# Robinatp/YOLO_Tensorflow

Measured on AMD Instinct MI355X. Metric: images_per_sec, higher is better.
Workload: dtype bf16; 1 GPU; YOLOv3 416x416 batch=32 per GPU, bf16: conv stack + head decode + threshold + TF-NMS; global_batch=32, input=uint8 NHWC resident in HBM, weights=seeded synthetic darknet stream (seed 0), parallelism=dp1

## Files before the change

yolo_tensorflow_amd/csrc/kernels.h:

```cpp
#pragma once
#ifndef OUT_STORE_AUX
#define OUT_STORE_AUX 16
#endif
#ifndef HALO_LOAD_AUX
#define HALO_LOAD_AUX 0
#endif
#ifndef RES_LOAD_AUX
#define RES_LOAD_AUX 0
#endif
#include <hip/hip_runtime.h>
#include <stdint.h>
typedef unsigned out_u32x4 __attribute__((ext_vector_type(4)));
__device__ __forceinline__ void out_store16_at(const void *base, unsigned byte_off, unsigned x, unsigned y, unsigned z, unsigned w)
{
#if defined(__HIP_DEVICE_COMPILE__)
    __amdgpu_buffer_rsrc_t r = __builtin_amdgcn_make_buffer_rsrc((void *)base, 0, 0x80000000u, 0x00020000);
    __builtin_amdgcn_raw_buffer_store_b128(out_u32x4{x, y, z, w}, r, byte_off, 0, OUT_STORE_AUX);
#endif
}

typedef uint16_t bf16_t;
struct fp8_t { uint8_t b; };
struct f16_t { uint16_t b; };
enum { DT_BF16 = 0, DT_F32 = 1, DT_FP8 = 2, DT_F16 = 3 };
// ... 88 lines not shown
};
bool conv_stem_pair_ok(const StemPairArgs &a);
hipError_t launch_conv_stem_pair(const StemPairArgs &a, hipStream_t s);
bool conv_c8_direct_pair_ok(const ConvArgs &a);
hipError_t launch_conv_c8_direct_pair(const ConvArgs &a, hipStream_t s);
hipError_t launch_conv_fp8(const ConvArgs &a, int cfg, hipStream_t s);
hipError_t launch_conv_diag(const ConvArgs &a, hipStream_t s);
struct StemArgs {
    const void *in; int in_stride;
    const uint8_t *in_u8; float in_scale, in_mul, in_add;
    const void *w0; const float *b0; int Kpad0, C0, act0;
    const void *w1; const float *b1; int Kpad1, C1, act1;
    void *out; int out_stride;
    int dt;
    const void *w2; const float *b2; int Kpad2, C2, act2;
    void *out2; int out2_stride;
    int N, H, W, Ho, Wo;
    const void *zeros;
};
bool conv_stem_ok(const StemArgs &a);
hipError_t launch_conv_stem(const StemArgs &a, hipStream_t s);
struct HaloArgs {
    const void *in; int in_stride;
    const void *w; const float *b; int Kpad, Cin, Cout, act;
    const void *res; int res_stride;
    void *out; int out_stride;
    int N, H, W;
    int dt;
};
bool conv_halo_ok(const HaloArgs &a);
hipError_t launch_conv_halo(const HaloArgs &a, hipStream_t s);
bool conv_s2_ok(const HaloArgs &a);
hipError_t launch_conv_s2(const HaloArgs &a, hipStream_t s);
struct BlockArgs {
    const void *x; int x_stride;
    const void *w1; const float *b1; int Kpad1, act1;
    const void *w2; const float *b2; int Kpad2, act2;
    void *out; int out_stride;
    int N, H, W, C, Cmid;
    int dt;
};
bool conv_resblock_ok(const BlockArgs &a);
hipError_t launch_conv_resblock(const BlockArgs &a, hipStream_t s);
hipError_t launch_conv_f32(const ConvArgs &a, hipStream_t s);

hipError_t launch_preprocess(const void *img, int fmt , int n, int hw, float scale,
                             void *out, int out_dt, int out_stride, hipStream_t s, float post_mul = 1.0f, float post_add = 0.0f);
hipError_t launch_resize_u8(const uint8_t *img, int h, int w, int s_out, void *out, int out_dt,
                            int out_stride, int out_c, hipStream_t s, float post_scale = 1.0f, float post_add = 0.0f);
hipError_t launch_resize_cv2_u8(const uint8_t *img, int h, int w, int oh, int ow, int swap_rb, float divisor, float *out, hipStream_t s);
struct ImgDesc { unsigned long long offset; int h, w; };
enum { FIT_STRETCH = 0, FIT_LETTERBOX = 1, FIT_CV2 = 2, FIT_CV2_BGR = 3 };
hipError_t launch_fit_images(const uint8_t *pixels, size_t bytes, const ImgDesc *d_descs, int n, int fit, int S, void *out, int out_dt,
                             int out_stride, float post_mul, float post_add, hipStream_t s);
__host__ __device__ inline void letterbox_dims(int netw, int neth, int w, int h, int *new_w, int *new_h)
{
    if (((float)netw / w) < ((float)neth / h)) { *new_w = netw; *new_h = (h * netw) / w; } else { *new_h = neth; *new_w = (w * neth) / h; }
}
__host__ __device__ inline float fit_unit_value(int fit, unsigned v)
{
    if (fit == FIT_STRETCH) return (float)v / 255.0f;
    if (fit == FIT_LETTERBOX) return (float)((double)v / 255.);
    return (float)v;
}
hipError_t launch_upsample2x(const TView &in, const TView &out, int bilinear, hipStream_t s);
hipError_t launch_maxpool(const TView &in, const TView &out, int size, int stride, int pad, hipStream_t s);
// ... 82 lines not shown
```

yolo_tensorflow_amd/csrc/yolo_api.cpp:

```cpp
#include "yolo_ctx.h"

extern "C" {

yolo_ctx *yolo_create(const yolo_config *cfg, char *err, size_t err_len)
{
    auto bail = [&](yolo_ctx *c, const std::string &m) -> yolo_ctx * { if (err && err_len) snprintf(err, err_len, "%s", m.c_str()); if (c) yolo_destroy(c); return nullptr; };
    if (!cfg || cfg->struct_size != sizeof(yolo_config)) return bail(nullptr, "yolo_create: bad yolo_config (struct_size)");
    if (cfg->max_batch < 1) return bail(nullptr, "yolo_create: max_batch < 1");
    if (cfg->dtype != YOLO_BF16 && cfg->dtype != YOLO_FP32 && cfg->dtype != YOLO_FP8 && cfg->dtype != YOLO_FP16 && cfg->dtype != YOLO_FP16X2) return bail(nullptr, "yolo_create: dtype");
    yolo_ctx *c = new yolo_ctx();
    c->device = cfg->device; c->max_batch = cfg->max_batch; c->dtype = cfg->dtype; c->semantics = cfg->semantics;
    c->decode = cfg->decode; c->keep_layers = cfg->keep_layers;
    int ndev = 0;
    if (hipGetDeviceCount(&ndev) != hipSuccess || ndev < 1) return bail(c, "yolo_create: no HIP device (this library has no CPU fallback)");
    if (hipSetDevice(c->device) != hipSuccess) return bail(c, "yolo_create: hipSetDevice failed");
    if (cfg->stream) c->stream = (hipStream_t)cfg->stream;
    else { if (hipStreamCreate(&c->stream) != hipSuccess) return bail(c, "yolo_create: hipStreamCreate failed"); c->own_stream = true; }
    std::vector<Section> secs; std::string perr;
    c->cfg_text = cfg->cfg_text ? cfg->cfg_text : "";
    if (!parse_cfg(cfg->cfg_text, secs, perr)) return bail(c, perr);
    if (build_plan(c, secs) != YOLO_OK) return bail(c, c->err);
    if (allocate(c) != YOLO_OK) return bail(c, c->err);
    resolve_scales(c);
    return c;
// ... 17 lines not shown

const char *yolo_last_error(const yolo_ctx *c) { return c ? c->err.c_str() : g_op_err.c_str(); }

size_t yolo_weights_count(const yolo_ctx *c) { return c ? c->weights_count : 0; }

int yolo_input_size(const yolo_ctx *c, int *h, int *w, int *ch) { if (!c) return YOLO_ERR_INVALID; if (h) *h = c->in_h; if (w) *w = c->in_w; if (ch) *ch = c->in_c; return YOLO_OK; }
int yolo_num_rows(const yolo_ctx *c) { return c ? c->rows : YOLO_ERR_INVALID; }
int yolo_num_attrs(const yolo_ctx *c) { return c ? c->attrs : YOLO_ERR_INVALID; }
int yolo_num_classes(const yolo_ctx *c) { return !c ? YOLO_ERR_INVALID : c->cls_layer >= 0 ? c->layers[c->cls_layer].C : c->attrs - 5; }
int yolo_num_layers(const yolo_ctx *c) { return c ? (int)c->layers.size() : YOLO_ERR_INVALID; }
int yolo_head_geometry(const yolo_ctx *c, int head, int *kind, int *grid, int *anchors, int *row_offset)
{
    if (!c || head < 0) return YOLO_ERR_INVALID;
    int k = 0;
    for (auto &L : c->layers) {
        if (L.type != L_YOLO && L.type != L_REGION && L.type != L_DETECT) continue;
        if (k++ != head) continue;
        if (kind) *kind = L.type == L_REGION ? 1 : L.type == L_DETECT ? 2 : 0;
        if (grid) *grid = L.H;
        if (anchors) *anchors = L.na;
        if (row_offset) *row_offset = L.row_off;
        return YOLO_OK;
    }
    return YOLO_ERR_INVALID;
}
double yolo_conv_flops(const yolo_ctx *c) { return c ? c->conv_flops : 0; }
double yolo_conv_bytes(const yolo_ctx *c, int n)
{
    if (!c) return 0;
    double b = 0;
    for (auto &L : c->layers) if (L.type == L_CONV) {
        TView in = view_of(c, L.in[0]);
        const double ie = (double)dt_size(L.in_dt), oe = (double)dt_size(L.out.dt);
        if (!L.stem && !L.stem_tail && !L.blk) b += (double)n * in.h * in.w * L.cin * ie;
        if (!L.stem_skip && !L.blk_skip && !L.pstem_skip) b += (double)n * L.H * L.W * L.filters * oe;
        b += (double)L.filters * L.cin * L.size * L.size * ie;
    }
    return b;
}

int yolo_darknet_boxes(yolo_ctx *c, int w, int h, float thresh, int relative, float *records, int cap, int *count)
{
    return yolo_darknet_boxes_at(c, 0, w, h, thresh, relative, records, cap, count);
}

int yolo_darknet_boxes_at(yolo_ctx *c, int image, int w, int h, float thresh, int relative, float *records, int cap, int *count)
{
    if (!c || !count) return YOLO_ERR_INVALID;
    if (int r = need_detector(c, "yolo_darknet_boxes")) return r;
    if (c->last_n < 1 || !c->det_valid) return fail(c, YOLO_ERR_STATE, "yolo_darknet_boxes needs a yolo_forward* pass first");
    if (image < 0 || image >= c->last_n) return fail(c, YOLO_ERR_INVALID, "image %d outside the last forward's batch of %d", image, c->last_n);
    if (w < 1 || h < 1 || cap < 0 || (cap > 0 && !records)) return fail(c, YOLO_ERR_INVALID, "bad image size / capacity");
    HIPCK(c, hipSetDevice(c->device));
    if (!c->d_dn_rec) {
        HIPCK(c, hipMalloc((void **)&c->d_dn_rec, (size_t)c->rows * c->attrs * 4));
        HIPCK(c, hipMalloc((void **)&c->d_dn_src, (size_t)c->rows * 4));
        HIPCK(c, hipMalloc((void **)&c->d_dn_count, 4));
    }
    DnBoxesArgs a; memset(&a, 0, sizeof a);
    a.det = c->d_det + (size_t)image * c->rows * c->attrs; a.attrs = c->attrs;
    for (size_t li = 0; li < c->layers.size(); ++li) {
        const Layer &L = c->layers[li];
        if (L.type != L_YOLO && L.type != L_REGION && L.type != L_DETECT) continue;
        if (a.nheads == 8) return fail(c, YOLO_ERR_UNSUPPORTED, "more than 8 heads");
        if (L.type == L_DETECT) {
            if (a.nheads) return fail(c, YOLO_ERR_UNSUPPORTED, "a [detection] head next to other heads");
            a.raw = (const float *)c->layers[li - 1].out.ptr + (size_t)image * c->layers[li - 1].out.stride; a.side = L.side; a.classes = L.classes; a.sqr = L.sqr;
            a.kind[0] = 2; a.grid[0] = L.side; a.na[0] = L.na; a.off[0] = L.row_off; a.nheads = 1;
// ... 58 lines not shown
    HIPCK(c, hipMemcpyAsync(out, c->d_dn_last, need * 4, hipMemcpyDeviceToHost, c->stream)); HIPCK(c, hipStreamSynchronize(c->stream));
    return YOLO_OK;
}

int yolo_last_layer_output(yolo_ctx *c, float *out, size_t out_floats) { return yolo_last_layer_output_batch(c, 1, out, out_floats); }

int yolo_head_raw(yolo_ctx *c, int head, int n, float *out, size_t out_floats)
{
    if (!c || !out || head < 0) return YOLO_ERR_INVALID;
    if (int r = need_detector(c, "yolo_head_raw")) return r;
    if (c->last_n < 1 || n < 1 || n > c->last_n) return fail(c, YOLO_ERR_STATE, "yolo_head_raw of %d images but the last forward ran %d", n, c->last_n);
    int k = 0;
    for (size_t li = 1; li < c->layers.size(); ++li) {
        const Layer &L = c->layers[li];
        if (L.type != L_YOLO && L.type != L_REGION && L.type != L_DETECT) continue;
        if (k++ != head) continue;
        const Layer &P = c->layers[li - 1];
        const size_t px = (size_t)n * P.H * P.W, need = px * P.C;
        if (out_floats < need) return fail(c, YOLO_ERR_INVALID, "output buffer too small (%zu < %zu floats)", out_floats, need);
        if (P.out.dt != DT_F32 || !P.out.ptr) return fail(c, YOLO_ERR_STATE, "internal: head conv output is not fp32");
        HIPCK(c, hipSetDevice(c->device));
        HIPCK(c, hipMemcpy2DAsync(out, (size_t)P.C * 4, P.out.ptr, (size_t)P.out.stride * 4, (size_t)P.C * 4, px, hipMemcpyDeviceToHost, c->stream));
        HIPCK(c, hipStreamSynchronize(c->stream));
        return YOLO_OK;
    }
    return fail(c, YOLO_ERR_INVALID, "no detection head %d", head);
}

int yolo_synchronize(yolo_ctx *c) { if (!c) return YOLO_ERR_INVALID; HIPCK(c, hipStreamSynchronize(c->stream)); return YOLO_OK; }

int yolo_layer_output(yolo_ctx *c, int index, int n, float *out, size_t out_floats, int *dims_out)
{
    if (!c) return YOLO_ERR_INVALID;
    if (!c->keep_layers) return fail(c, YOLO_ERR_STATE, "yolo_layer_output needs keep_layers=1");
    if (index < 0 || index >= (int)c->layers.size() || n < 1 || n > c->last_n) return fail(c, YOLO_ERR_INVALID, "bad layer index / n");
    const Layer &L = c->layers[index];
    if (dims_out) { dims_out[0] = L.H; dims_out[1] = L.W; dims_out[2] = L.C; }
    size_t need = (size_t)n * L.H * L.W * L.C;
    if (!out) return YOLO_OK;
    if (out_floats < need) return fail(c, YOLO_ERR_INVALID, "output buffer too small");
    HIPCK(c, hipSetDevice(c->device));
    float *tmp = nullptr; HIPCK(c, hipMalloc((void **)&tmp, need * 4));
    TView v = L.out; v.n = n;
    float vs = 1.f;
    if (v.dt == DT_FP8) {
        vs = c->eff_scale[index];
        if (vs != vs) { hipFree(tmp); return fail(c, YOLO_ERR_UNSUPPORTED, "layer %d concatenates tensors with different fp8 scales; read its sources", index); }
    }
    hipError_t e = hipSuccess;
    float *wide = nullptr;
    if (L.pair && v.dt == DT_F16) {
        const int cp = roundup(L.C, 32);
        e = hipMalloc((void **)&wide, (size_t)n * L.H * L.W * cp * 4);
        if (e == hipSuccess) e = launch_split_to_f32(v.ptr, v.stride, cp, wide, cp, (size_t)n * L.H * L.W, c->stream);
        v.ptr = wide; v.stride = cp; v.dt = DT_F32;
    }
    if (e == hipSuccess) e = launch_to_f32(v, tmp, c->stream, vs);
    if (e == hipSuccess) e = hipMemcpyAsync(out, tmp, need * 4, hipMemcpyDeviceToHost, c->stream);
    if (e == hipSuccess) e = hipStreamSynchronize(c->stream);
    hipFree(tmp); if (wide) hipFree(wide);
    if (e != hipSuccess) return fail(c, YOLO_ERR_HIP, "layer_output: %s", hipGetErrorString(e));
    return YOLO_OK;
}

}
```

yolo_tensorflow_amd/csrc/yolo_ctx.h:

```cpp
#pragma once
#include "../../include/yolo_hip.h"
#include "kernels.h"

#include <algorithm>
#include <cmath>
#include <cstdarg>
#include <cstdio>
#include <cstdlib>
#include <cstring>
#include <map>
#include <string>
#include <vector>

namespace yolo_impl {

enum LType { L_CONV, L_SHORTCUT, L_ROUTE, L_UPSAMPLE, L_MAXPOOL, L_REORG, L_YOLO, L_REGION, L_DETECT, L_LOCAL, L_AVGPOOL, L_SOFTMAX };

struct Section { std::string type; std::map<std::string, std::string> kv; };

struct Layer {
    LType type;
    int H = 0, W = 0, C = 0;
    std::vector<int> in;
    int filters = 0, size = 0, stride = 1, pad = 0, bn = 0, act = ACT_LINEAR;
    int cin = 0, cin_pad = 0, kpad = 0, cout_pad = 0;
    void *d_w = nullptr; float *d_b = nullptr; float *d_sc = nullptr;
    void *d_wf = nullptr;
    int in_dt = DT_BF16;
    int store_dt = DT_BF16;
    bool pair = false;
    int tile_cfg = -1;
    int residual_from = -2;
    bool head = false;
    float *d_obj = nullptr;
    bool stem_skip = false, stem = false;
    bool pstem_skip = false, pstem = false;
    bool blk_skip = false, blk = false;
    bool stem_tail = false;
    bool halo = false;
    bool s2 = false;
    bool fc = false; int fc_h = 0, fc_w = 0, fc_c = 0;
    bool s2d7 = false;
    int side = 0, sqr = 0;
    int tail_layer = -1, fused_into = -1; bool tail_on = false;
    bool noop = false;
    std::vector<int> copy_inputs;
    std::vector<int> copy_offsets;
    int psize = 0, pstride = 0, ppad = 0;
    int na = 0, classes = 0, row_off = 0;
    std::vector<float> anchors;
    int groups = 1; float temperature = 1.f; bool pool_fused = false; bool cost = false;
    int storage = -1; int ch_off = 0;
    TView out;
};

struct Storage { int def = 1 << 30, last = -1; size_t bytes = 0; int phys = -1; int stride = 0; int dt = DT_BF16; bool persistent = false; };


}
using namespace yolo_impl;

struct yolo_ctx {
    std::string err, cfg_text;
    int device = 0;
    hipStream_t stream = nullptr; bool own_stream = false;
    int max_batch = 1, dtype = YOLO_BF16, semantics = YOLO_SEM_TF, decode = YOLO_DECODE_RATIO, keep_layers = 0;
    int in_h = 0, in_w = 0, in_c = 0;
    std::vector<Layer> layers;
    std::vector<Storage> storages;
    std::vector<void *> phys; std::vector<size_t> phys_bytes;
    TView input;
    void *d_zeros = nullptr;
    void *d_stage = nullptr; size_t stage_bytes = 0;
// ... 82 lines not shown
```

yolo_tensorflow_amd/csrc/yolo_plan.cpp:

```cpp
#include "yolo_ctx.h"

namespace yolo_impl {

bool parse_cfg(const char *text, std::vector<Section> &out, std::string &err)
{
    std::string s(text ? text : "");
    size_t pos = 0;
    while (pos <= s.size()) {
        size_t e = s.find('\n', pos); if (e == std::string::npos) e = s.size();
        std::string line = s.substr(pos, e - pos); pos = e + 1;
        size_t a = line.find_first_not_of(" \t\r"); if (a == std::string::npos) continue;
        size_t b = line.find_last_not_of(" \t\r"); line = line.substr(a, b - a + 1);
        if (line[0] == '#' || line[0] == ';') continue;
        if (line[0] == '[') {
            size_t r = line.find(']'); if (r == std::string::npos) { err = "cfg: unterminated section " + line; return false; }
            Section sec; sec.type = line.substr(1, r - 1); out.push_back(sec);
        } else {
            size_t eq = line.find('='); if (eq == std::string::npos || out.empty()) { err = "cfg: bad line '" + line + "'"; return false; }
            std::string k = line.substr(0, eq), v = line.substr(eq + 1);
            auto trim = [](std::string &t) { size_t x = t.find_first_not_of(" \t"); size_t y = t.find_last_not_of(" \t"); t = x == std::string::npos ? "" : t.substr(x, y - x + 1); };
            trim(k); trim(v); out.back().kv[k] = v;
        }
    }
    if (out.empty() || (out[0].type != "net" && out[0].type != "network")) { err = "cfg: first section must be [net]"; return false; }
// ... 221 lines not shown
        }
    if (ctx16 && !c->keep_layers && NL >= 2 && (double)c->max_batch * c->in_h * c->in_w * 8 * 2 < 2147483648.0) {
        const Layer &A = c->layers[0], &B = c->layers[1];
        if (A.type == L_CONV && B.type == L_CONV && uses[0] == 1 && B.in[0] == 0 && A.size == 3 && A.stride == 1 && A.pad == 1 && A.cin == 3 &&
            A.filters == 32 && B.size == 3 && B.stride == 2 && B.pad == 1 && B.filters == 64 && !A.head && !B.head && B.residual_from < -1 &&
            is16(A.in_dt) && A.store_dt == A.in_dt && B.in_dt == A.in_dt && B.store_dt == A.in_dt && !c->in_pair && !A.pair && !B.pair) {
            c->layers[0].stem_skip = true; c->layers[1].stem = true;
            if (NL >= 3) {
                const Layer &T = c->layers[2];
                if (T.type == L_CONV && !T.fc && T.in[0] == 1 && T.size == 1 && T.stride == 1 && T.pad == 0 && T.filters == 32 && !T.head && T.residual_from < -1 &&
                    T.in_dt == A.in_dt && T.store_dt == A.in_dt && !T.pair)
                    c->layers[2].stem_tail = true;
            }
        }
    }
    if (c->split() && !c->keep_layers && NL >= 2 && c->in_pair && !getenv("YOLO_NO_PAIR_STEM")) {
        const Layer &A = c->layers[0], &B = c->layers[1];
        if (A.type == L_CONV && B.type == L_CONV && uses[0] == 1 && B.in[0] == 0 && A.size == 3 && A.stride == 1 && A.pad == 1 && A.cin == 3 && A.bn == B.bn &&
            (A.filters == 32) && B.size == 3 && B.stride == 2 && B.pad == 1 && B.filters == 64 && !A.head && !B.head && A.residual_from < -1 && B.residual_from < -1 &&
            A.pair && B.pair && c->in_h % 2 == 0 && c->in_w % 2 == 0 && A.kpad >= 216 && B.kpad == 576) {
            c->layers[0].pstem_skip = true; c->layers[1].pstem = true;
        }
    }
    if (ctx16 && !getenv("YOLO_NO_HALO"))
        for (int i = 1; i < NL; ++i) {
            Layer &L = c->layers[i];
            if (L.type == L_CONV && !L.head && !L.stem && !L.stem_skip && !L.stem_tail && !L.blk && L.size == 3 && L.stride == 1 && L.pad == 1 && L.cin == 32 && L.filters == 64 &&
                is16(L.in_dt) && L.store_dt == L.in_dt && (L.residual_from < 0 || c->layers[L.residual_from].store_dt == L.in_dt) && !L.pair && !c->pair_of(L.in[0]))
                L.halo = true;
            if (L.type == L_CONV && !L.head && !L.stem && !L.stem_skip && !L.stem_tail && !L.blk && !L.blk_skip && L.size == 3 && L.stride == 2 && L.pad == 1 && L.cin == 64 &&
                L.filters == 128 && L.residual_from < -1 && is16(L.in_dt) && L.store_dt == L.in_dt && !L.pair && !c->pair_of(L.in[0]) && !getenv("YOLO_NO_S2"))
                L.s2 = true;
        }
    if (ctx16 && !c->keep_layers) {
        for (int i = 0; i + 1 < NL; ++i) {
            Layer &P = c->layers[i];
            if (P.type != L_CONV || P.fc || P.head || P.stem || P.stem_skip || P.stem_tail || P.blk || P.s2 || P.halo || (P.filters != 128 && P.filters != 256)) continue;
            if (c->split() && (P.pair || c->pair_of(P.in[0]))) continue;
            int o = i;
            if (P.residual_from >= -1) o = i + 1;
            const int j = o + 1;
            if (j >= NL) continue;
            Layer &T = c->layers[j];
            if (T.type == L_CONV && !T.fc && T.in[0] == o && T.size == 1 && T.stride == 1 && T.pad == 0 && T.filters * 2 == P.filters && !T.head &&
                T.residual_from < -1 && !T.stem_tail && !T.blk_skip && T.in_dt == P.in_dt && !T.pair) { P.tail_layer = j; T.fused_into = i; }
            else if (T.type == L_CONV && !T.fc && T.head && T.in[0] == o && uses[o] == 1 && T.size == 1 && T.stride == 1 && T.pad == 0 && P.filters == 256 && T.filters <= 256 &&
                     P.size == 3 && P.residual_from < -1 && T.act == ACT_LINEAR && T.in_dt == P.in_dt && (T.in_dt == DT_BF16 || T.in_dt == DT_F16) && j + 1 < NL && c->layers[j + 1].type == L_YOLO) { P.tail_layer = j; T.fused_into = i; }
        }
    }
    std::vector<int> place_route(NL, -1), place_off(NL, 0);
    for (int i = 0; i < NL; ++i) {
        Layer &L = c->layers[i];
        if (L.type != L_ROUTE || L.in.size() < 2) continue;
        int off = 0;
        for (int j : L.in) {
            int cj = j < 0 ? c->in_c : c->layers[j].C;
            const int gran = L.pair ? 32 : gran_of(L.store_dt);
            bool ok = j >= 0 && place_route[j] < 0 && c->layers[j].type != L_ROUTE && !c->layers[j].head &&
                      c->layers[j].type != L_YOLO && c->layers[j].type != L_REGION && c->layers[j].type != L_DETECT && (cj % gran == 0) && (off % gran == 0) &&
                      c->layers[j].type != L_SOFTMAX && !c->layers[j].cost && !(c->layers[j].type == L_AVGPOOL && c->layers[j].store_dt != L.store_dt);
            if (ok && c->layers[j].type == L_CONV && j + 1 < NL && c->layers[j + 1].noop && c->layers[j + 1].type == L_SHORTCUT) ok = false;
            if (ok) { place_route[j] = i; place_off[j] = L.pair ? 2 * off : off; }
            else { L.copy_inputs.push_back(j); L.copy_offsets.push_back(off); }
            off += cj;
        }
    }
// ... 2 lines not shown
        c->storages.push_back(s); return (int)c->storages.size() - 1;
    };
    for (int i = 0; i < NL; ++i) {
        Layer &L = c->layers[i];
        if (L.type == L_ROUTE && L.in.size() >= 2) {
            L.storage = new_storage(L.pair ? pair_width(L.C) : roundup(L.C, gran_of(L.store_dt)), L.store_dt, (size_t)c->max_batch * L.H * L.W, c->keep_layers); L.ch_off = 0;
        }
    }
    for (int i = 0; i < NL; ++i) {
        Layer &L = c->layers[i];
        if (L.type == L_YOLO || L.type == L_REGION || L.type == L_DETECT) { L.noop = true; L.storage = c->layers[i - 1].storage; L.ch_off = c->layers[i - 1].ch_off; continue; }
        if (L.type == L_ROUTE && L.in.size() == 1) { L.noop = true; int j = L.in[0]; if (j < 0) return fail(c, YOLO_ERR_UNSUPPORTED, "route to network input"); L.storage = c->layers[j].storage; L.ch_off = c->layers[j].ch_off; continue; }
        if (L.type == L_ROUTE) continue;
        if (L.stem_skip || L.pstem_skip) { L.noop = true; continue; }
        if (L.type == L_SOFTMAX) { L.storage = new_storage(L.C, DT_F32, (size_t)c->max_batch, true); continue; }
        if (place_route[i] >= 0) { L.storage = c->layers[place_route[i]].storage; L.ch_off = place_off[i]; }
        else if (L.head) L.storage = new_storage(roundup(L.C, 4), DT_F32, (size_t)c->max_batch * L.H * L.W, true);
        else L.storage = new_storage(L.pair ? pair_width(L.C) : roundup(L.C, gran_of(L.store_dt)), L.store_dt, (size_t)c->max_batch * L.H * L.W, c->keep_layers);
    }
    for (int i = 0; i + 1 < NL; ++i) {
        Layer &L = c->layers[i];
        if (L.type == L_CONV && L.residual_from >= -1) {
            Storage &mine = c->storages[L.storage];
            if (place_route[i] < 0) mine.bytes = 0;
            L.storage = c->layers[i + 1].storage; L.ch_off = c->layers[i + 1].ch_off;
        }
    }
    for (int i = 0; i < NL; ++i) {
        Layer &L = c->layers[i];
        if (L.storage < 0) continue;
        if (!L.noop) { Storage &s = c->storages[L.storage]; s.def = std::min(s.def, L.fused_into >= 0 ? L.fused_into : i); s.last = std::max(s.last, i); }
        for (int j : L.in) if (j >= 0 && c->layers[j].storage >= 0) { Storage &s = c->storages[c->layers[j].storage]; s.last = std::max(s.last, i); }
        if (L.type == L_CONV && L.residual_from >= 0) { Storage &s = c->storages[c->layers[L.residual_from].storage]; s.last = std::max(s.last, i); }
    }
    std::vector<int> free_list;
    for (int i = 0; i < NL; ++i) {
        for (size_t k = 0; k < c->storages.size(); ++k) {
            Storage &s = c->storages[k];
            if (s.def != i || s.bytes == 0) continue;
            int pick = -1;
            if (!s.persistent) {
                for (size_t f = 0; f < free_list.size(); ++f)
                    if (pick < 0 || c->phys_bytes[free_list[f]] > c->phys_bytes[free_list[pick]]) pick = (int)f;
            }
            if (pick >= 0) { s.phys = free_list[pick]; free_list.erase(free_list.begin() + pick); c->phys_bytes[s.phys] = std::max(c->phys_bytes[s.phys], s.bytes); }
            else { s.phys = (int)c->phys_bytes.size(); c->phys_bytes.push_back(s.bytes); }
        }
        for (size_t k = 0; k < c->storages.size(); ++k) {
            Storage &s = c->storages[k];
            if (s.last == i && s.phys >= 0 && !s.persistent) free_list.push_back(s.phys);
        }
    }
    return YOLO_OK;
}

int allocate(yolo_ctx *c)
{
    c->phys.assign(c->phys_bytes.size(), nullptr);
    for (size_t i = 0; i < c->phys_bytes.size(); ++i) {
        HIPCK(c, hipMalloc(&c->phys[i], c->phys_bytes[i] + 256));
        HIPCK(c, hipMemsetAsync(c->phys[i], 0, c->phys_bytes[i] + 256, c->stream));
    }
    for (auto &L : c->layers) {
        L.out.n = c->max_batch; L.out.h = L.H; L.out.w = L.W; L.out.c = L.C;
        if (L.storage < 0) continue;
        Storage &s = c->storages[L.storage];
// ... 55 lines not shown
    HIPCK(c, hipMalloc((void **)&c->d_scores, nr * 4)); HIPCK(c, hipMalloc((void **)&c->d_labels, nr * 4));
    HIPCK(c, hipMalloc((void **)&c->d_cand, nr * 4)); HIPCK(c, hipMalloc((void **)&c->d_keys, (size_t)c->max_batch * c->rows_pow2 * 8));
    HIPCK(c, hipMalloc((void **)&c->d_sbox, nr * 16)); HIPCK(c, hipMalloc((void **)&c->d_slabel, nr * 4)); HIPCK(c, hipMalloc((void **)&c->d_sscore, nr * 4));
    HIPCK(c, hipMalloc((void **)&c->d_counts, (size_t)c->max_batch * 4));
    for (auto &L : c->layers) if (L.type == L_CONV) {
        size_t wb = (size_t)L.cout_pad * L.kpad * dt_size(L.in_dt);
        HIPCK(c, hipMalloc(&L.d_w, wb)); HIPCK(c, hipMemsetAsync(L.d_w, 0, wb, c->stream));
        HIPCK(c, hipMalloc((void **)&L.d_b, (size_t)L.cout_pad * 4)); HIPCK(c, hipMemsetAsync(L.d_b, 0, (size_t)L.cout_pad * 4, c->stream));
        if (L.in_dt == DT_FP8) { HIPCK(c, hipMalloc((void **)&L.d_sc, (size_t)L.cout_pad * 4)); HIPCK(c, hipMemsetAsync(L.d_sc, 0, (size_t)L.cout_pad * 4, c->stream)); }
    }
    for (auto &L : c->layers) if (L.type == L_LOCAL) {
        const size_t wn = (size_t)L.H * L.W * L.filters * L.size * L.size * L.cin;
        HIPCK(c, hipMalloc(&L.d_w, wn * dt_size(L.in_dt))); HIPCK(c, hipMalloc((void **)&L.d_b, (size_t)L.H * L.W * L.filters * 4));
    }
    if (c->dtype != YOLO_FP32)
        for (size_t i = 1; i < c->layers.size(); ++i) {
            const Layer &Y = c->layers[i]; Layer &P = c->layers[i - 1];
            if (Y.type == L_YOLO && P.type == L_CONV && P.head && !P.fc) HIPCK(c, hipMalloc((void **)&P.d_obj, (size_t)c->max_batch * P.H * P.W * Y.na * 4));
        }
    HIPCK(c, hipStreamSynchronize(c->stream));
    if (c->dtype != YOLO_FP32)
        for (size_t i = 0; i < c->layers.size(); ++i) {
            const Layer &L = c->layers[i];
            if (L.type != L_CONV || L.fc || L.s2d7 || L.stem_skip || L.stem || L.stem_tail || L.blk_skip || L.pstem_skip || L.pstem) continue;
            const TView in = view_of(c, L.in[0]);
            const double per_image = (double)in.h * in.w * in.stride * dt_size(L.in_dt), slack = 2.0 * (in.w + 1) * in.stride * dt_size(L.in_dt);
            if (per_image * c->max_batch + slack >= 2147483648.0)
                return fail(c, YOLO_ERR_UNSUPPORTED, "max_batch %d: layer %zu reads %.0f bytes per image%s, and a conv's whole-batch input must stay below 2 GiB (32-bit buffer offsets): at most %d images per context",
                            c->max_batch, i, per_image, c->split() ? " (split fp16 pairs: 2 x the channels)" : "", (int)((2147483648.0 - slack - 1) / per_image));
        }
    return YOLO_OK;
}

bool fixed_kernel(const Layer &L) { return L.stem || L.stem_skip || L.stem_tail || L.halo || L.s2 || L.blk || L.blk_skip || L.pstem || L.pstem_skip; }

}
```

yolo_tensorflow_amd/csrc/yolo_run.cpp:

```cpp
#include "yolo_ctx.h"

namespace yolo_impl {

int fail(yolo_ctx *c, int code, const char *fmt, ...)
{
    char buf[512];
    va_list ap; va_start(ap, fmt); vsnprintf(buf, sizeof buf, fmt, ap); va_end(ap);
    if (c) c->err = buf;
    return code;
}

ConvArgs conv_args(const yolo_ctx *c, const Layer &L, int n)
{
    ConvArgs a; memset(&a, 0, sizeof a);
    TView in = view_of(c, L.in[0]);
    a.in = in.ptr; a.in_stride = in.stride; a.wt = L.d_w; a.bias = L.d_b;
    a.out = L.out.ptr; a.out_stride = L.out.stride; a.out_dt = L.out.dt; a.in_dt = L.in_dt; a.oscale = L.d_sc;
    if (L.pair || (c->split() && L.out.dt == DT_F32)) a.split = 1;
    a.pairk = L.in[0] >= 0 && c->pair_of(L.in[0]) ? 1 : 0;
    a.out_inv_scale = 1.f; a.res_scale = 1.f; a.mid_scale = 1.f; a.mid_inv_scale = 1.f;
    const int li = (int)(&L - c->layers.data());
    if (L.residual_from >= -1) { TView r = view_of(c, L.residual_from); a.res = r.ptr; a.res_stride = r.stride; }
    if (L.tail_on && L.tail_layer >= 0 && c->layers[L.tail_layer].in_dt == L.in_dt && (L.in_dt == DT_FP8 || c->layers[L.tail_layer].d_wf)) {
        const Layer &T = c->layers[L.tail_layer];
// ... 54 lines not shown
            t.in = c->input.ptr; t.w0 = A.d_w; t.b0 = A.d_b; t.Kpad0 = A.kpad; t.C0 = A.filters; t.act0 = A.act;
            t.in_u8 = c->stem_u8; t.in_scale = c->stem_scale; t.in_mul = c->in_mul; t.in_add = c->in_add;
            t.w1 = L.d_w; t.b1 = L.d_b; t.Kpad1 = L.kpad; t.act1 = L.act;
            t.out = L.out.ptr; t.out_stride = L.out.stride; t.N = n; t.H = A.H; t.W = A.W; t.Ho = L.H; t.Wo = L.W;
            if (c->input.stride != 24 || !conv_stem_pair_ok(t)) return fail(c, YOLO_ERR_STATE, "layer %d: the fused split-fp16 stem does not apply to this plan", i);
            HIPCK(c, launch_conv_stem_pair(t, s));
            break;
        }
        if (L.fused_into >= 0 && c->layers[L.fused_into].tail_on) break;
        if (L.stem) {
            const Layer &A = c->layers[0];
            StemArgs t; memset(&t, 0, sizeof t);
            t.in = c->input.ptr; t.in_stride = c->input.stride;
            t.in_u8 = c->stem_u8; t.in_scale = c->stem_scale; t.in_mul = c->in_mul; t.in_add = c->in_add;
            t.w0 = A.d_w; t.b0 = A.d_b; t.Kpad0 = A.kpad; t.C0 = A.filters; t.act0 = A.act;
            t.w1 = L.d_w; t.b1 = L.d_b; t.Kpad1 = L.kpad; t.C1 = L.filters; t.act1 = L.act;
            if (i + 1 < (int)c->layers.size() && c->layers[i + 1].stem_tail) {
                const Layer &T = c->layers[i + 1];
                t.w2 = T.d_w; t.b2 = T.d_b; t.Kpad2 = T.kpad; t.C2 = T.filters; t.act2 = T.act; t.out2 = T.out.ptr; t.out2_stride = T.out.stride;
            }
            t.out = L.out.ptr; t.out_stride = L.out.stride; t.N = n; t.H = A.H; t.W = A.W; t.Ho = L.H; t.Wo = L.W; t.zeros = c->d_zeros; t.dt = L.in_dt;
            HIPCK(c, launch_conv_stem(t, s));
            break;
        }
        if (L.blk_skip || L.blk) {
            const Layer &A = L.blk ? c->layers[i - 1] : L, &B = L.blk ? L : c->layers[i + 1];
            const TView x = view_of(c, A.in[0]);
            BlockArgs b; memset(&b, 0, sizeof b);
            b.x = x.ptr; b.x_stride = x.stride; b.w1 = A.d_w; b.b1 = A.d_b; b.Kpad1 = A.kpad; b.act1 = A.act;
            b.w2 = B.d_w; b.b2 = B.d_b; b.Kpad2 = B.kpad; b.act2 = B.act; b.out = B.out.ptr; b.out_stride = B.out.stride;
            b.N = n; b.H = B.H; b.W = B.W; b.C = B.filters; b.Cmid = A.filters; b.dt = B.in_dt;
            if (conv_resblock_ok(b)) {
                if (L.blk) HIPCK(c, launch_conv_resblock(b, s));
                break;
            }
        }
        ConvArgs a = conv_args(c, L, n);
        if (L.tail_on && !a.w2) return fail(c, YOLO_ERR_STATE, "layer %d: the plan folds the 1x1 conv %d into this layer, but its filters are not available in the producer's operand type", i, L.tail_layer);
        if (L.s2d7) HIPCK(c, launch_reorg(nview(c->input), nview(c->s2d), 2, 0, s));
        if (L.halo) {
            HaloArgs h; memset(&h, 0, sizeof h);
            h.in = a.in; h.in_stride = a.in_stride; h.w = a.wt; h.b = a.bias; h.Kpad = a.Kpad; h.Cin = L.cin; h.Cout = L.filters; h.act = L.act;
            h.res = a.res; h.res_stride = a.res_stride; h.out = a.out; h.out_stride = a.out_stride; h.N = n; h.H = L.H; h.W = L.W; h.dt = L.in_dt;
            if (conv_halo_ok(h)) { HIPCK(c, launch_conv_halo(h, s)); break; }
        }
        if (L.s2) {
            HaloArgs h; memset(&h, 0, sizeof h);
            const TView in = view_of(c, L.in[0]);
            h.in = a.in; h.in_stride = a.in_stride; h.w = a.wt; h.b = a.bias; h.Kpad = a.Kpad; h.Cin = L.cin; h.Cout = L.filters; h.act = L.act;
            h.res = a.res; h.out = a.out; h.out_stride = a.out_stride; h.N = n; h.H = in.h; h.W = in.w; h.dt = L.in_dt;
            if (conv_s2_ok(h)) { HIPCK(c, launch_conv_s2(h, s)); break; }
        }
        if (c->dtype == YOLO_FP32) { HIPCK(c, launch_conv_f32(a, s)); break; }
        const int cfg = conv_resolve_cfg(a, L.tile_cfg);
        if (a.w2 && !a.split && !a.pairk && !conv_cfg_tail_ok(cfg, a.Cout, a.in_dt == DT_FP8, a.tail_f32 != 0)) return fail(c, YOLO_ERR_STATE, "layer %d: tile config %d cannot run the fused 1x1 tail", i, cfg);
        HIPCK(c, a.in_dt == DT_FP8 ? launch_conv_fp8(a, cfg, s) : launch_conv_bf16(a, cfg, s));
        break; }
    case L_SHORTCUT:
        if (!L.noop && L.pair) {
            HIPCK(c, launch_add_split(view_of(c, L.in[0]).ptr, view_of(c, L.in[0]).stride, view_of(c, L.in[1]).ptr, view_of(c, L.in[1]).stride, L.out.ptr, L.out.stride, roundup(L.C, 32), (size_t)n * L.H * L.W, s));
        } else if (!L.noop) {
            float sa = 1.f, sb = 1.f, so = 1.f;
            if (c->dtype == YOLO_FP8) { sa = c->eff_scale[L.in[0]]; sb = c->eff_scale[L.in[1]]; so = 1.f / c->eff_scale[i]; }
            HIPCK(c, launch_add(nview(view_of(c, L.in[0])), nview(view_of(c, L.in[1])), nview(L.out), s, sa, sb, so));
        }
        break;
// ... 568 lines not shown
```

Baseline: 13040 img/s.

## Fuse residual 3x3 conv and following stride-2 downsample conv into one kernel

Adds a persistent, warp-specialized kernel that computes the 3x3 conv (32->64 with residual add) into an LDS tile and immediately feeds it to the next 3x3 stride-2 conv (64->128). Producer waves stream input and residual via buffer-load-to-LDS with triple buffering while consumer waves run the downsampling conv and store output. The planner enables it when keep_layers is off and the pattern matches. This removes the HBM round trip of the intermediate 208x208x64 tensor and one launch, at the cost of recomputing halo pixels and heavy LDS use that limits occupancy. Also relaxes yolo_layer_output to allow non-reused conv buffers without keep_layers.

New measurement: 13210 img/s, median of 6. +1.3%, better.

```diff
diff --git a/yolo_tensorflow_amd/csrc/conv_c3s2.hip b/yolo_tensorflow_amd/csrc/conv_c3s2.hip
--- /dev/null
+++ b/yolo_tensorflow_amd/csrc/conv_c3s2.hip
@@ -0,0 +1,248 @@
+#include "kernels.h"
+#include "device_common.h"
+
+constexpr int CS_TH = 4, CS_TW = 8;
+constexpr int CS_LH = 2 * CS_TH + 1, CS_LW = 2 * CS_TW + 1;
+constexpr int CS_LPIX = CS_LH * CS_LW;
+constexpr int CS_GROUPS = (CS_LPIX + 15) / 16;
+[[maybe_unused]] constexpr int CS_NG = (CS_GROUPS + 3) / 4;
+constexpr int CS_PITCH = 144;
+constexpr int CS_L4_CHUNKS = (CS_LPIX * (CS_PITCH / 16) + 63) / 64;
+constexpr int CS_L4_BYTES = CS_L4_CHUNKS * 1024;
+[[maybe_unused]] constexpr int CS_L4_K = (CS_L4_CHUNKS + 3) / 4;
+constexpr int CS_IH = CS_LH + 2, CS_IW = CS_LW + 2;
+constexpr int CS_INPIX = CS_IH * CS_IW;
+constexpr int CS_IN_CHUNKS = (CS_INPIX * 4 + 63) / 64;
+constexpr int CS_IN_BYTES = CS_IN_CHUNKS * 1024;
+[[maybe_unused]] constexpr int CS_IN_K = (CS_IN_CHUNKS + 3) / 4;
+constexpr int CS_OPITCH = 128 * 2 + 16;
+constexpr int CS_OUT_BYTES = CS_TH * CS_TW * CS_OPITCH;
+constexpr int CS_NW = 8;
+constexpr size_t CS_LDS = (size_t)3 * CS_L4_BYTES + 2 * CS_IN_BYTES + 2 * CS_OUT_BYTES;
+static_assert(((CS_GROUPS * 16 - 1) / CS_LW + 2) * CS_IW + (CS_GROUPS * 16 - 1) % CS_LW + 2 < CS_IN_CHUNKS * 16, "conv3: reads past the layer-2 window slot");
+
+template <bool H16>
+__global__ __launch_bounds__(64 * CS_NW) void conv_c3s2_c32_c64_c128(const C3S2Args a)
+{
+#if defined(__HIP_DEVICE_COMPILE__)
+    extern __shared__ __attribute__((aligned(16))) char smem[];
+    if constexpr (H16) fp16_saturating_mode();
+    const int tid = threadIdx.x, lane = tid & 63, wave = __builtin_amdgcn_readfirstlane(tid >> 6);
+    const int l15 = lane & 15, lq = lane >> 4;
+    const int sub = wave & 3;
+
+    const int Ho = (a.H - 1) / 2 + 1, Wo = (a.W - 1) / 2 + 1;
+    const int tiles_x = (Wo + CS_TW - 1) / CS_TW, tiles_y = (Ho + CS_TH - 1) / CS_TH;
+    const int per_img = tiles_x * tiles_y, ntiles = a.N * per_img;
+    const int G = (int)gridDim.x;
+    const int nt = (ntiles - (int)blockIdx.x + G - 1) / G;
+    struct TilePos { int n, ty, tx; };
+    auto tile_pos = [&](int j) { const int tile = (int)blockIdx.x + j * G; TilePos q; q.n = tile / per_img; const int tr = tile - q.n * per_img; q.ty = tr / tiles_x; q.tx = tr - q.ty * tiles_x; return q; };
+
+    char *const l4b = smem, *const inb = smem + 3 * CS_L4_BYTES, *const lob = inb + 2 * CS_IN_BYTES;
+
+    if (wave < 4) {
+        bf16x8 fw[4][9];
+#pragma unroll
+        for (int ct = 0; ct < 4; ++ct)
+#pragma unroll
+            for (int t = 0; t < 9; ++t)
+                fw[ct][t] = *(const bf16x8 *)((const bf16_t *)a.w3 + (size_t)(ct * 16 + l15) * a.Kpad3 + t * 32 + lq * 8);
+        f32x4 bv[4];
+#pragma unroll
+        for (int ct = 0; ct < 4; ++ct) bv[ct] = *(const f32x4 *)(a.b3 + ct * 16 + lq * 4);
+        const float slope = a.act3 == ACT_LEAKY ? 0.1f : 1.f;
+        __amdgpu_buffer_rsrc_t rin = buf_rsrc(a.in);
+        __amdgpu_buffer_rsrc_t rres = buf_rsrc(a.res);
+
+        unsigned relr[CS_L4_K]; int wyxr[CS_L4_K];
+#pragma unroll
+        for (int k = 0; k < CS_L4_K; ++k) {
+            const int g = (sub + 4 * k) * 64 + lane;
+            const int px = g / 9, j = g - px * 9;
+            const int wy = px / CS_LW, wx = px - wy * CS_LW;
+            const bool valid = px < CS_LPIX && j < 8;
+            relr[k] = (unsigned)(((wy * a.W + wx) * a.res_stride + ((j ^ ((wy >> 1) & 1)) * 8)) * 2);
+            wyxr[k] = valid ? (wy | (wx << 8)) : -1;
+        }
+        unsigned reli[CS_IN_K]; int wyxi[CS_IN_K];
+#pragma unroll
+        for (int k = 0; k < CS_IN_K; ++k) {
+            const int g = (sub + 4 * k) * 64 + lane;
+            const int px = g >> 2, pc = g & 3;
+            const int ry = px / CS_IW, rx = px - ry * CS_IW;
+            const int sc = pc ^ (2 * ((px >> 2) & 1));
+            reli[k] = (unsigned)(((ry * a.W + rx) * a.in_stride + sc * 8) * 2);
+            wyxi[k] = px < CS_INPIX ? (ry | (rx << 8)) : -1;
+        }
+        auto produce = [&](int jf, int jc, char *__restrict__ l4_fill, char *__restrict__ in_fill, const char *__restrict__ in_cur, char *__restrict__ l4) {
+            if (jf < nt) {
+                const TilePos q = tile_pos(jf);
+                const int iy0 = 2 * q.ty * CS_TH - 1, ix0 = 2 * q.tx * CS_TW - 1;
+                const unsigned baser = (unsigned)(((q.n * a.H + iy0) * a.W + ix0) * a.res_stride * 2);
+                const unsigned basei = (unsigned)(((q.n * a.H + iy0 - 1) * a.W + ix0 - 1) * a.in_stride * 2);
+#pragma unroll
+                for (int k = 0; k < CS_L4_K; ++k) {
+                    const int c = sub + 4 * k;
+                    if (c < CS_L4_CHUNKS) {
+                        const int wy = wyxr[k] & 0xff, wx = (wyxr[k] >> 8) & 0xff;
+                        const bool ok = wyxr[k] >= 0 && (unsigned)(iy0 + wy) < (unsigned)a.H && (unsigned)(ix0 + wx) < (unsigned)a.W;
+                        __builtin_amdgcn_raw_ptr_buffer_load_lds(rres, (lds_void *)(l4_fill + c * 1024), 16, ok ? baser + relr[k] : 0x80000000u, 0, 0, 0);
+                    }
+                }
+#pragma unroll
+                for (int k = 0; k < CS_IN_K; ++k) {
+                    const int c = sub + 4 * k;
+                    if (c < CS_IN_CHUNKS) {
+                        const int ry = wyxi[k] & 0xff, rx = (wyxi[k] >> 8) & 0xff;
+                        const bool ok = wyxi[k] >= 0 && (unsigned)(iy0 - 1 + ry) < (unsigned)a.H && (unsigned)(ix0 - 1 + rx) < (unsigned)a.W;
+                        __builtin_amdgcn_raw_ptr_buffer_load_lds(rin, (lds_void *)(in_fill + c * 1024), 16, ok ? basei + reli[k] : 0x80000000u, 0, 0, 0);
+                    }
+                }
+            }
+            if (jc < nt) {
+                const TilePos q = tile_pos(jc);
+                const int iy0 = 2 * q.ty * CS_TH - 1, ix0 = 2 * q.tx * CS_TW - 1;
+                int l15s = l15, lqs = lq;
+                asm volatile("" : "+v"(l15s), "+v"(lqs));
+#pragma unroll
+                for (int jj = 0; jj < CS_NG; ++jj) {
+                    const int g = sub + 4 * jj;
+                    if (g < CS_GROUPS) {
+                        const int idx = g * 16 + l15s;
+                        const int ly = (idx * 3856) >> 16;
+                        const int lx = idx - ly * CS_LW;
+                        const int p0 = ly * CS_IW + lx;
+                        f32x4 acc[4];
+#pragma unroll
+                        for (int ct = 0; ct < 4; ++ct) acc[ct] = f32x4{0.f, 0.f, 0.f, 0.f};
+#pragma unroll
+                        for (int t = 0; t < 9; ++t) {
+                            const int kh = t / 3, kw = t - kh * 3;
+                            const int p = p0 + kh * CS_IW + kw;
+                            const bf16x8 x = *(const bf16x8 *)(in_cur + p * 64 + ((lqs ^ (2 * ((p >> 2) & 1))) << 4));
+#pragma unroll
+                            for (int ct = 0; ct < 4; ++ct) acc[ct] = mma16<H16>(fw[ct][t], x, acc[ct]);
+                        }
+                        const bool inside = (unsigned)(iy0 + ly) < (unsigned)a.H && (unsigned)(ix0 + lx) < (unsigned)a.W;
+                        char *const rec = l4 + (ly * CS_LW + lx) * CS_PITCH + (lqs & 1) * 8;
+                        const int swz = (ly >> 1) & 1;
+                        if (idx < CS_LPIX) {
+#pragma unroll
+                            for (int ct = 0; ct < 4; ++ct) {
+                                uint2 *const q4 = (uint2 *)(rec + (((ct * 2 + (lqs >> 1)) ^ swz) << 4));
+                                const uint2 r = *q4;
+                                const uint2 pk = leaky_pack4<H16>(acc[ct], bv[ct], slope);
+                                uint2 o;
+                                o.x = pack16x2<H16>(unpack16_lo<H16>(pk.x) + unpack16_lo<H16>(r.x), unpack16_hi<H16>(pk.x) + unpack16_hi<H16>(r.x));
+                                o.y = pack16x2<H16>(unpack16_lo<H16>(pk.y) + unpack16_lo<H16>(r.y), unpack16_hi<H16>(pk.y) + unpack16_hi<H16>(r.y));
+                                o.x = inside ? o.x : 0u; o.y = inside ? o.y : 0u;
+                                *q4 = o;
+                            }
+                        }
+                    }
+                }
+            }
+        };
+        if (nt > 0) produce(0, nt, l4b, inb, inb + CS_IN_BYTES, l4b + CS_L4_BYTES);
+        __builtin_amdgcn_s_waitcnt(waitcnt_imm(0, 0));
+        __builtin_amdgcn_s_barrier();
+        for (int i = -1, c3 = 0, par = 0; i <= nt; ++i, c3 = c3 == 2 ? 0 : c3 + 1, par ^= 1) {
+            const int f3 = c3 == 2 ? 0 : c3 + 1;
+            produce(i + 2, i + 1, l4b + f3 * CS_L4_BYTES, inb + (par ^ 1) * CS_IN_BYTES, inb + par * CS_IN_BYTES, l4b + c3 * CS_L4_BYTES);
+            __builtin_amdgcn_s_waitcnt(waitcnt_imm(0, 0));
+            __builtin_amdgcn_s_barrier();
+        }
+    } else {
+        const int grp = sub;
+        bf16x8 fw[2][18];
+#pragma unroll
+        for (int ct = 0; ct < 2; ++ct)
+#pragma unroll
+            for (int ks = 0; ks < 18; ++ks)
+                fw[ct][ks] = *(const bf16x8 *)((const bf16_t *)a.w5 + (size_t)(grp * 32 + ct * 16 + l15) * a.Kpad5 + ks * 32 + lq * 8);
+        f32x4 bv[2];
+#pragma unroll
+        for (int ct = 0; ct < 2; ++ct) bv[ct] = *(const f32x4 *)(a.b5 + grp * 32 + ct * 16 + lq * 4);
+        const float slope = a.act5 == ACT_LEAKY ? 0.1f : 1.f;
+        const int ctid = tid - 256;
+        int pb[2];
+#pragma unroll
+        for (int sb = 0; sb < 2; ++sb) {
+            const int r = 2 * sb + (l15 >> 3), c = l15 & 7;
+            pb[sb] = ((2 * r) * CS_LW + 2 * c) * CS_PITCH;
+        }
+        const int rpar = (l15 >> 3) & 1;
+        auto consume = [&](int jprev, int jcur, const char *__restrict__ lo_prev, const char *__restrict__ l4, char *__restrict__ lo) {
+            if (jprev >= 0) {
+                const TilePos q = tile_pos(jprev);
+                const int oy0 = q.ty * CS_TH, ox0 = q.tx * CS_TW;
+#pragma unroll
+                for (int it = 0; it < CS_TH * CS_TW * 16 / 256; ++it) {
+                    const int c = ctid + it * 256;
+                    const int px = c >> 4, chunk = c & 15;
+                    const int oy = oy0 + (px >> 3), ox = ox0 + (px & 7);
+                    const uint4 o = *(const uint4 *)(lo_prev + px * CS_OPITCH + chunk * 16);
+                    const unsigned so = (oy < Ho && ox < Wo) ? (unsigned)((((size_t)(q.n * Ho + oy) * Wo + ox) * a.out_stride + chunk * 8) * 2) : 0x80000000u;
+                    out_store16_at(a.out, so, o.x, o.y, o.z, o.w);
+                }
+            }
+            if (jcur >= 0 && jcur < nt) {
+                f32x4 acc[2][2];
+#pragma unroll
+                for (int sb = 0; sb < 2; ++sb)
+#pragma unroll
+                    for (int ct = 0; ct < 2; ++ct) acc[sb][ct] = f32x4{0.f, 0.f, 0.f, 0.f};
+#pragma unroll
+                for (int t = 0; t < 9; ++t) {
+                    const int kh = t / 3, kw = t - kh * 3;
+                    const int swz = rpar ^ (kh >> 1);
+#pragma unroll
+                    for (int hh = 0; hh < 2; ++hh) {
+                        const int coff = ((hh * 4 + lq) ^ swz) << 4;
+#pragma unroll
+                        for (int sb = 0; sb < 2; ++sb) {
+                            const bf16x8 x = *(const bf16x8 *)(l4 + pb[sb] + (kh * CS_LW + kw) * CS_PITCH + coff);
+#pragma unroll
+                            for (int ct = 0; ct < 2; ++ct) acc[sb][ct] = mma16<H16>(fw[ct][t * 2 + hh], x, acc[sb][ct]);
+                        }
+                    }
+                }
+#pragma unroll
+                for (int sb = 0; sb < 2; ++sb)
+#pragma unroll
+                    for (int ct = 0; ct < 2; ++ct)
+                        *(uint2 *)(lo + (sb * 16 + l15) * CS_OPITCH + (grp * 32 + ct * 16 + lq * 4) * 2) = leaky_pack4<H16>(acc[sb][ct], bv[ct], slope);
+            }
+        };
+        __builtin_amdgcn_s_waitcnt(waitcnt_imm(63, 0));
+        __builtin_amdgcn_s_barrier();
+        for (int i = -1, c3 = 0, par = 0; i <= nt; ++i, c3 = c3 == 2 ? 0 : c3 + 1, par ^= 1) {
+            const int u3 = c3 == 0 ? 2 : c3 - 1;
+            consume(i >= 1 ? i - 1 : -1, i, lob + par * CS_OUT_BYTES, l4b + u3 * CS_L4_BYTES, lob + (par ^ 1) * CS_OUT_BYTES);
+            __builtin_amdgcn_s_waitcnt(waitcnt_imm(63, 0));
+            __builtin_amdgcn_s_barrier();
+        }
+    }
+#endif
+}
+
+bool conv_c3s2_ok(const C3S2Args &a)
+{
+    const double pin = (double)a.N * a.H * a.W, pout = (double)a.N * ((a.H - 1) / 2 + 1) * ((a.W - 1) / 2 + 1);
+    if (pin * a.in_stride * 2.0 >= 2147483648.0 || pin * a.res_stride * 2.0 >= 2147483648.0 || pout * a.out_stride * 2.0 >= 2147483648.0) return false;
+    return (a.dt == DT_BF16 || a.dt == DT_F16) && a.in && a.res && a.out && a.Kpad3 >= 288 && a.Kpad5 >= 576 && a.N >= 1 && a.H >= 2 && a.W >= 2 &&
+           (a.in_stride % 8) == 0 && a.in_stride >= 32 && (a.res_stride % 8) == 0 && a.res_stride >= 64 && (a.out_stride % 8) == 0 && a.out_stride >= 128;
+}
+hipError_t launch_conv_c3s2(const C3S2Args &a, hipStream_t s)
+{
+    if (!conv_c3s2_ok(a)) return hipErrorInvalidValue;
+    const bool h16 = a.dt == DT_F16;
+    { hipError_t e = conv_opt_in_lds(h16 ? (const void *)conv_c3s2_c32_c64_c128<true> : (const void *)conv_c3s2_c32_c64_c128<false>, CS_LDS); if (e != hipSuccess) return e; }
+    const int Ho = (a.H - 1) / 2 + 1, Wo = (a.W - 1) / 2 + 1;
+    const long tiles = (long)a.N * ((Wo + CS_TW - 1) / CS_TW) * ((Ho + CS_TH - 1) / CS_TH);
+    long blocks = 256; if (blocks > tiles) blocks = tiles;
+    if (h16) hipLaunchKernelGGL(conv_c3s2_c32_c64_c128<true>, dim3((unsigned)blocks), dim3(64 * CS_NW), CS_LDS, s, a);
+    else hipLaunchKernelGGL(conv_c3s2_c32_c64_c128<false>, dim3((unsigned)blocks), dim3(64 * CS_NW), CS_LDS, s, a);
+    return hipGetLastError();
+}
diff --git a/yolo_tensorflow_amd/csrc/kernels.h b/yolo_tensorflow_amd/csrc/kernels.h
--- a/yolo_tensorflow_amd/csrc/kernels.h
+++ b/yolo_tensorflow_amd/csrc/kernels.h
@@ -144,6 +144,17 @@
 hipError_t launch_conv_halo(const HaloArgs &a, hipStream_t s);
 bool conv_s2_ok(const HaloArgs &a);
 hipError_t launch_conv_s2(const HaloArgs &a, hipStream_t s);
+struct C3S2Args {
+    const void *in; int in_stride;
+    const void *w3; const float *b3; int Kpad3, act3;
+    const void *res; int res_stride;
+    const void *w5; const float *b5; int Kpad5, act5;
+    void *out; int out_stride;
+    int N, H, W;
+    int dt;
+};
+bool conv_c3s2_ok(const C3S2Args &a);
+hipError_t launch_conv_c3s2(const C3S2Args &a, hipStream_t s);
 struct BlockArgs {
     const void *x; int x_stride;
     const void *w1; const float *b1; int Kpad1, act1;
diff --git a/yolo_tensorflow_amd/csrc/yolo_api.cpp b/yolo_tensorflow_amd/csrc/yolo_api.cpp
--- a/yolo_tensorflow_amd/csrc/yolo_api.cpp
+++ b/yolo_tensorflow_amd/csrc/yolo_api.cpp
@@ -73,8 +73,8 @@
     for (auto &L : c->layers) if (L.type == L_CONV) {
         TView in = view_of(c, L.in[0]);
         const double ie = (double)dt_size(L.in_dt), oe = (double)dt_size(L.out.dt);
-        if (!L.stem && !L.stem_tail && !L.blk) b += (double)n * in.h * in.w * L.cin * ie;
-        if (!L.stem_skip && !L.blk_skip && !L.pstem_skip) b += (double)n * L.H * L.W * L.filters * oe;
+        if (!L.stem && !L.stem_tail && !L.blk && !L.c3s2) b += (double)n * in.h * in.w * L.cin * ie;
+        if (!L.stem_skip && !L.blk_skip && !L.pstem_skip && !L.c3s2_skip) b += (double)n * L.H * L.W * L.filters * oe;
         b += (double)L.filters * L.cin * L.size * L.size * ie;
     }
     return b;
@@ -199,9 +199,13 @@
 int yolo_layer_output(yolo_ctx *c, int index, int n, float *out, size_t out_floats, int *dims_out)
 {
     if (!c) return YOLO_ERR_INVALID;
-    if (!c->keep_layers) return fail(c, YOLO_ERR_STATE, "yolo_layer_output needs keep_layers=1");
     if (index < 0 || index >= (int)c->layers.size() || n < 1 || n > c->last_n) return fail(c, YOLO_ERR_INVALID, "bad layer index / n");
     const Layer &L = c->layers[index];
+    if (!c->keep_layers) {
+        bool kept = L.type == L_CONV && L.storage >= 0 && L.residual_from < -1 && !L.stem_skip && !L.pstem_skip && !L.blk_skip && !L.c3s2_skip;
+        if (kept) for (const Storage &o : c->storages) if (&o != &c->storages[L.storage] && o.phys == c->storages[L.storage].phys && o.def > c->storages[L.storage].def) kept = false;
+        if (!kept) return fail(c, YOLO_ERR_STATE, "yolo_layer_output needs keep_layers=1 (without it: only a conv layer's own tensor whose buffer no later layer reuses)");
+    }
     if (dims_out) { dims_out[0] = L.H; dims_out[1] = L.W; dims_out[2] = L.C; }
     size_t need = (size_t)n * L.H * L.W * L.C;
     if (!out) return YOLO_OK;
diff --git a/yolo_tensorflow_amd/csrc/yolo_ctx.h b/yolo_tensorflow_amd/csrc/yolo_ctx.h
--- a/yolo_tensorflow_amd/csrc/yolo_ctx.h
+++ b/yolo_tensorflow_amd/csrc/yolo_ctx.h
@@ -39,6 +39,7 @@
     bool stem_tail = false;
     bool halo = false;
     bool s2 = false;
+    bool c3s2_skip = false, c3s2 = false;
     bool fc = false; int fc_h = 0, fc_w = 0, fc_c = 0;
     bool s2d7 = false;
     int side = 0, sqr = 0;
diff --git a/yolo_tensorflow_amd/csrc/yolo_plan.cpp b/yolo_tensorflow_amd/csrc/yolo_plan.cpp
--- a/yolo_tensorflow_amd/csrc/yolo_plan.cpp
+++ b/yolo_tensorflow_amd/csrc/yolo_plan.cpp
@@ -277,6 +277,12 @@
                 L.filters == 128 && L.residual_from < -1 && is16(L.in_dt) && L.store_dt == L.in_dt && !L.pair && !c->pair_of(L.in[0]) && !getenv("YOLO_NO_S2"))
                 L.s2 = true;
         }
+    if (ctx16 && !c->keep_layers && !getenv("YOLO_NO_C3S2"))
+        for (int i = 1; i + 2 < NL; ++i) {
+            Layer &A = c->layers[i], &S = c->layers[i + 1], &B = c->layers[i + 2];
+            if (A.halo && B.s2 && A.residual_from >= 0 && S.type == L_SHORTCUT && S.noop && uses[i] == 1 && uses[i + 1] == 1 && B.in[0] == i + 1 && A.in[0] >= 0 &&
+                A.in_dt == B.in_dt && c->layers[A.residual_from].C == 64) { A.c3s2_skip = true; B.c3s2 = true; }
+        }
     if (ctx16 && !c->keep_layers) {
         for (int i = 0; i + 1 < NL; ++i) {
             Layer &P = c->layers[i];
@@ -345,6 +351,10 @@
         if (!L.noop) { Storage &s = c->storages[L.storage]; s.def = std::min(s.def, L.fused_into >= 0 ? L.fused_into : i); s.last = std::max(s.last, i); }
         for (int j : L.in) if (j >= 0 && c->layers[j].storage >= 0) { Storage &s = c->storages[c->layers[j].storage]; s.last = std::max(s.last, i); }
         if (L.type == L_CONV && L.residual_from >= 0) { Storage &s = c->storages[c->layers[L.residual_from].storage]; s.last = std::max(s.last, i); }
+        if (L.c3s2) {
+            const Layer &A = c->layers[i - 2];
+            for (int j : {A.in[0], A.residual_from}) if (j >= 0 && c->layers[j].storage >= 0) { Storage &s = c->storages[c->layers[j].storage]; s.last = std::max(s.last, i); }
+        }
     }
     std::vector<int> free_list;
     for (int i = 0; i < NL; ++i) {
@@ -466,6 +476,6 @@
     return YOLO_OK;
 }
 
-bool fixed_kernel(const Layer &L) { return L.stem || L.stem_skip || L.stem_tail || L.halo || L.s2 || L.blk || L.blk_skip || L.pstem || L.pstem_skip; }
+bool fixed_kernel(const Layer &L) { return L.stem || L.stem_skip || L.stem_tail || L.halo || L.s2 || L.blk || L.blk_skip || L.pstem || L.pstem_skip || L.c3s2 || L.c3s2_skip; }
 
 }
diff --git a/yolo_tensorflow_amd/csrc/yolo_run.cpp b/yolo_tensorflow_amd/csrc/yolo_run.cpp
--- a/yolo_tensorflow_amd/csrc/yolo_run.cpp
+++ b/yolo_tensorflow_amd/csrc/yolo_run.cpp
@@ -110,6 +110,18 @@
             b.N = n; b.H = B.H; b.W = B.W; b.C = B.filters; b.Cmid = A.filters; b.dt = B.in_dt;
             if (conv_resblock_ok(b)) {
                 if (L.blk) HIPCK(c, launch_conv_resblock(b, s));
+                break;
+            }
+        }
+        if (L.c3s2_skip || L.c3s2) {
+            const Layer &A = L.c3s2 ? c->layers[i - 2] : L, &B = L.c3s2 ? L : c->layers[i + 2];
+            const TView x = view_of(c, A.in[0]), r = view_of(c, A.residual_from);
+            C3S2Args t; memset(&t, 0, sizeof t);
+            t.in = x.ptr; t.in_stride = x.stride; t.w3 = A.d_w; t.b3 = A.d_b; t.Kpad3 = A.kpad; t.act3 = A.act; t.res = r.ptr; t.res_stride = r.stride;
+            t.w5 = B.d_w; t.b5 = B.d_b; t.Kpad5 = B.kpad; t.act5 = B.act; t.out = B.out.ptr; t.out_stride = B.out.stride;
+            t.N = n; t.H = A.H; t.W = A.W; t.dt = B.in_dt;
+            if (conv_c3s2_ok(t)) {
+                if (L.c3s2) HIPCK(c, launch_conv_c3s2(t, s));
                 break;
             }
         }
```
